# aoschu/esn-ofdm-mimo

Measured on AMD Instinct MI355X. Metric: OFDM symbols/s through the ESN detector (4x8 TDL-B, N=128, N_res=512; train+predict+detect), higher is better.
Workload: dtype f16 operands / f32 accumulate

## Files before the change

esn_ofdm_mimo_amd/build.py:

```python
import os
import subprocess
import sys

PKG = os.path.dirname(os.path.abspath(__file__))
CSRC = os.path.join(PKG, "csrc")
LIB = os.path.join(PKG, "libesn_hip.so")
SOURCES = ["esn_api.hip", "esn_host.hip", "esn_pack.hip", "esn_recur_f64.hip", "esn_recur_f64_mfma.hip", "esn_recur_mfma.hip",
           "esn_recur_big.hip", "esn_recur_cluster.hip", "esn_recur_mfma_f32.hip", "esn_recur_mfma_f16.hip", "esn_recur_mfma_bf16.hip", "esn_recur_skew16.hip", "esn_harvest_cluster.hip",
           "esn_solve_qr.hip", "esn_solve_chol.hip", "esn_solve_chol_big.hip", "esn_loo.hip", "esn_holdout.hip", "esn_gram.hip", "esn_detect.hip", "esn_remod.hip", "esn_gen.hip", "esn_reservoir.hip", "esn_specrad_split.hip", "esn_baseline.hip", "esn_chantrack.hip", "esn_chanstat.hip", "esn_coded.hip",
           "esn_elm.hip", "esn_fnn.hip"]
WITH_RS = os.environ.get("ESN_WITH_RS") == "1"
FLAGS = ["--offload-arch=gfx950", "-O3", "-std=c++17", "-fPIC", "-ffp-contract=off", "-fno-slp-vectorize",
         "-Wall", "-Wno-unused-function"]


def _stale():
    if not os.path.exists(LIB):
        return True
    t = os.path.getmtime(LIB)
    deps = [os.path.join(CSRC, f) for f in os.listdir(CSRC)] + \
           [os.path.join(PKG, "..", "include", "esn_hip.h"), os.path.abspath(__file__)]
    return any(os.path.getmtime(d) > t for d in deps)


def build_library(force=False, verbose=True, stamps=False):
    global LIB
    if stamps:
        extra = ["-DESN_STAMPS"] + os.environ.get("ESN_EXTRA_FLAGS", "").split()
        return _build(os.path.join(PKG, "libesn_hip_stamps.so"), "build_stamps", extra, verbose)
    if not force and not _stale():
        return LIB
    return _build(LIB, "build", [], verbose)


def _build(LIB, bdir, extra, verbose):
    hipcc = os.environ.get("HIPCC", "/opt/rocm/bin/hipcc")
    objs = []
    procs = []
    os.makedirs(os.path.join(PKG, bdir), exist_ok=True)
    sources = SOURCES + (["esn_recur_rs.hip"] if WITH_RS and LIB.endswith("_rs.so") else [])
    if len(sources) > len(SOURCES):
        extra = list(extra) + ["-DESN_WITH_RS"]
    for src in sources:
        obj = os.path.join(PKG, bdir, src.replace(".hip", ".o"))
        objs.append(obj)
        per_file = os.environ.get("ESN_FLAGS_" + src.replace(".hip", "").upper(), "").split()
        cmd = [hipcc, *FLAGS, *extra, *per_file, "-c", os.path.join(CSRC, src), "-o", obj]
        procs.append((src, subprocess.Popen(cmd, stdout=subprocess.PIPE, stderr=subprocess.STDOUT)))
    for src, pr in procs:
        out, _ = pr.communicate()
        if pr.returncode != 0:
            sys.stderr.write(out.decode())
            raise RuntimeError(f"hipcc failed on {src}")
        if verbose and out.strip():
            sys.stderr.write(out.decode())
    cmd = [hipcc, "--offload-arch=gfx950", "-shared", "-fPIC", "-o", LIB, *objs]
    subprocess.check_call(cmd)
    return LIB


if __name__ == "__main__":
    if "--variant" in sys.argv:
        name = sys.argv[sys.argv.index("--variant") + 1]
        print(_build(os.path.join(PKG, f"libesn_hip_{name}.so"), "build_" + name,
                     os.environ.get("ESN_EXTRA_FLAGS", "").split(), True))
    else:
        print(build_library(force="--force" in sys.argv, stamps="--stamps" in sys.argv))
```

esn_ofdm_mimo_amd/csrc/esn_api.hip:

```cpp
#include <stdarg.h>
#include <stdio.h>
#include <stdlib.h>
#include <math.h>
#include <string.h>
#include "esn_launch.h"
#include "esn_solve.h"

using namespace esn;

static thread_local char g_err[512] = "";

namespace esn {
int api_fail(int code, const char* fmt, ...) {
    va_list ap;
    va_start(ap, fmt);
    vsnprintf(g_err, sizeof(g_err), fmt, ap);
    va_end(ap);
    return code;
}
}
static int (&fail)(int, const char*, ...) = api_fail;

enum KnobRule {
    KNOB_FLAG,
    KNOB_INT,
    KNOB_TRIPLE,
    KNOB_BIG_NT,
    KNOB_HCLUSTER
};
struct KnobRow {
    const char* key;
    const char* env;
    size_t field;
    KnobRule rule;
    int dflt;
};
static const KnobRow kKnobTable[] = {
    {"skew", "ESN_SKEW", offsetof(Knobs, skew), KNOB_FLAG, 1},
    {"mfma_geom", "ESN_MFMA_GEOM", offsetof(Knobs, geom16), KNOB_TRIPLE, 0},
    {"mfma_geom_f32", "ESN_MFMA_GEOM_F32", offsetof(Knobs, geom32), KNOB_TRIPLE, 0},
    {"chol_skip", "ESN_CHOL_SKIP", offsetof(Knobs, chol_skip), KNOB_INT, 0},
    {"chol_dma", "ESN_CHOL_DMA", offsetof(Knobs, chol_dma), KNOB_FLAG, 1},
    {"f64_mfma", "ESN_F64_MFMA", offsetof(Knobs, f64_mfma), KNOB_FLAG, 1},
    {"rs", "ESN_RS", offsetof(Knobs, rs), KNOB_FLAG, 0},
    {"big_gemm", "ESN_BIG_GEMM", offsetof(Knobs, big_gemm), KNOB_FLAG, 1},
    {"cluster", "ESN_CLUSTER", offsetof(Knobs, cluster), KNOB_FLAG, 1},
    {"big_nt", "ESN_BIG_NT", offsetof(Knobs, big_nt), KNOB_BIG_NT, 2},
    {"big_pipe", "ESN_BIG_PIPE", offsetof(Knobs, big_pipe), KNOB_FLAG, 1},
    {"harvest_gemm", "ESN_HARVEST_GEMM", offsetof(Knobs, harvest_gemm), KNOB_FLAG, 0},
    {"gen_ko", nullptr, offsetof(Knobs, gen_ko), KNOB_INT, 0},
    {"s16", "ESN_S16", offsetof(Knobs, s16), KNOB_FLAG, 1},
    {"hcluster", "ESN_HCLUSTER", offsetof(Knobs, hcluster), KNOB_HCLUSTER, 1},
    {"detect_fixed", "ESN_DETECT_FIXED", offsetof(Knobs, detect_fixed), KNOB_FLAG, 1},
};

static void knob_parse(const KnobRow& r, const char* v, Knobs& k) {
    int* out = reinterpret_cast<int*>(reinterpret_cast<char*>(&k) + r.field);
    switch (r.rule) {
        case KNOB_FLAG: *out = (v && v[0] == '0' + !r.dflt) ? !r.dflt : r.dflt; break;
        case KNOB_INT: *out = v ? atoi(v) : r.dflt; break;
        case KNOB_TRIPLE: {
            int t[3];
            const bool ok = v && sscanf(v, "%d,%d,%d", &t[0], &t[1], &t[2]) == 3 && t[0] > 0 && t[1] > 0 && t[2] > 0;
            for (int i = 0; i < 3; ++i) out[i] = ok ? t[i] : 0;
            break;
        }
        case KNOB_BIG_NT: *out = (v && v[0] == '4') ? 4 : 2; break;
        case KNOB_HCLUSTER: *out = (v && (v[0] == '0' || v[0] == '4' || v[0] == '8')) ? v[0] - '0' : 1; break;
    }
}

namespace esn {
Knobs& knobs() {
    static Knobs k = [] {
        Knobs x{};
        for (const KnobRow& r : kKnobTable) knob_parse(r, r.env ? getenv(r.env) : nullptr, x);
        return x;
    }();
    return k;
}
}

static int hip_fail(int e, const char* what) {
    if (e == 0) return 0;
    if (e > 0) return fail(-1000 - e, "%s: HIP error %d (%s)", what, e, hipGetErrorString((hipError_t)e));
    return fail(-2, "%s: no kernel instance for this shape", what);
}

static bool check_shape(const esn_shape_t* s) {
    return s && s->n_res > 0 && s->n_in > 0 && s->n_out > 0 && s->n_wsets > 0;
}

static bool geometry_for(int precision, const esn_shape_t* s, Geometry* g, bool harvest = false) {
    memset(g, 0, sizeof(*g));
    if (precision == ESN_F64) {
        int fb = 8;
        while (fb > 1 && recur_f64_lds_bytes(fb, s->n_res, s->n_in, s->n_out) > 150 * 1024) fb >>= 1;
        if (recur_f64_lds_bytes(fb, s->n_res, s->n_in, s->n_out) > 160 * 1024) return false;
        Geometry gp, gh;
        memset(&gp, 0, sizeof(gp)); memset(&gh, 0, sizeof(gh));
        if (f64_mfma_geometry(s->n_res, s->n_in, s->n_out, false, &gp) &&
            f64_mfma_geometry(s->n_res, s->n_in, s->n_out, true, &gh))
            *g = harvest ? gh : gp;
        g->Bt = fb;
        return true;
    }
    if (precision < ESN_F64 || precision > ESN_BF16) return false;
    return mfma_geometry(precision, s->n_res, s->n_in, s->n_out, harvest, g);
}

#ifdef ESN_STAMPS
static unsigned long long* g_stamp_buf = nullptr;
extern "C" void esn_debug_set_stamp_buffer(void* dev) { g_stamp_buf = (unsigned long long*)dev; }
namespace esn { unsigned long long* stamp_buffer() { return g_stamp_buf; } }
#define ESN_SET_STAMPS(p) (p).stamps = g_stamp_buf
#else
#define ESN_SET_STAMPS(p) (p).stamps = nullptr
#endif

extern "C" {

const char* esn_last_error(void) { return g_err; }

int esn_abi_version(void) { return 10; }

int esn_debug_set(const char* key, const char* value) {
    if (!key) return fail(-1, "esn_debug_set: null key");
#ifndef ESN_WITH_RS
    if (!strcmp(key, "rs"))
        return (value && value[0] == '1')
                   ? fail(-3, "esn_debug_set: the register-state kernel is not in this build (ESN_WITH_RS=1)") : 0;
#endif
    for (const KnobRow& r : kKnobTable)
        if (!strcmp(key, r.key)) { knob_parse(r, value, knobs()); return 0; }
    return fail(-1, "esn_debug_set: unknown key '%s'", key);
}

int esn_device_info(int* cu_count, int* lds_bytes_per_cu, int* clock_khz, char* arch_name, int arch_name_len) {
    int dev = 0;
    hipError_t e = hipGetDevice(&dev);
    if (e != hipSuccess) return hip_fail((int)e, "hipGetDevice");
    hipDeviceProp_t prop;
    e = hipGetDeviceProperties(&prop, dev);
    if (e != hipSuccess) return hip_fail((int)e, "hipGetDeviceProperties");
    if (cu_count) *cu_count = prop.multiProcessorCount;
    if (lds_bytes_per_cu) *lds_bytes_per_cu = (int)prop.maxSharedMemoryPerMultiProcessor;
    if (clock_khz) *clock_khz = prop.clockRate;
    if (arch_name && arch_name_len > 0) {
        strncpy(arch_name, prop.gcnArchName, arch_name_len - 1);
        arch_name[arch_name_len - 1] = 0;
    }
    return 0;
}

int esn_tile_frames(int precision, const esn_shape_t* shape) {
    Geometry g;
    if (!check_shape(shape)) return fail(-1, "esn_tile_frames: invalid shape");
    if (!geometry_for(precision, shape, &g)) return fail(-2, "esn_tile_frames: unsupported shape/precision");
    return g.Bt;
}

size_t esn_packed_weights_bytes(int precision, const esn_shape_t* shape) {
    Geometry g;
    if (!check_shape(shape) || !geometry_for(precision, shape, &g)) return 0;
    return packed_w_bytes(precision, shape->n_res, shape->n_in, shape->n_out, g);
}

size_t esn_packed_readout_bytes(int precision, const esn_shape_t* shape) {
    Geometry g;
    if (!check_shape(shape) || !geometry_for(precision, shape, &g)) return 0;
    return packed_wout_bytes(precision, shape->n_res, shape->n_in, shape->n_out, g);
}

int esn_pack_weights(int precision, const esn_shape_t* shape, const double* W, const double* W_in,
                     const double* W_fb, void* packed, void* stream) {
    Geometry g;
    if (!check_shape(shape)) return fail(-1, "esn_pack_weights: invalid shape");
    if (!W || !W_in || !W_fb || !packed) return fail(-1, "esn_pack_weights: null pointer");
    if (!geometry_for(precision, shape, &g)) return fail(-2, "esn_pack_weights: unsupported shape/precision");
    return hip_fail(launch_pack_weights(precision, shape, g, W, W_in, W_fb, packed, (hipStream_t)stream),
                    "esn_pack_weights");
}

int esn_pack_readout(int precision, const esn_shape_t* shape, int n_groups, const double* W_out,
                     void* packed, void* stream) {
    Geometry g;
    if (!check_shape(shape) || n_groups <= 0) return fail(-1, "esn_pack_readout: invalid shape");
    if (!W_out || !packed) return fail(-1, "esn_pack_readout: null pointer");
    if (!geometry_for(precision, shape, &g)) return fail(-2, "esn_pack_readout: unsupported shape/precision");
    return hip_fail(launch_pack_readout(precision, shape, g, n_groups, W_out, packed, (hipStream_t)stream),
                    "esn_pack_readout");
}

static bool use_f64_mfma(int precision, const RecurParams& p) {
    return precision == ESN_F64 && p.g.m64 && p.n_frames > 8 && knobs().f64_mfma;
}

static int fill_common(RecurParams& p, int precision, const esn_shape_t* shape, const char* who,
                       bool harvest = false) {
    memset(&p, 0, sizeof(p));
    if (!check_shape(shape)) return fail(-1, "%s: invalid shape", who);
    if (!geometry_for(precision, shape, &p.g, harvest)) return fail(-2, "%s: unsupported shape/precision", who);
    p.n_res = shape->n_res; p.n_in = shape->n_in; p.n_out = shape->n_out;
    p.teacher_forcing = shape->teacher_forcing ? 1 : 0;
    p.n_wsets = shape->n_wsets;
    p.wset_stride = packed_w_bytes(precision, p.n_res, p.n_in, p.n_out, p.g);
    p.wout_stride = packed_wout_bytes(precision, p.n_res, p.n_in, p.n_out, p.g);
    p.leak = (shape->leak_rate == 0.0) ? 1.0 : shape->leak_rate;
    if (!(p.leak > 0.0 && p.leak <= 1.0)) return fail(-1, "%s: leak_rate %g outside (0, 1]", who, shape->leak_rate);
    if (p.leak != 1.0 && precision != ESN_F64)
        return fail(-2, "%s: leak_rate != 1 is an extension of the float64 kernels (precision ESN_F64)", who);
    p.w16_off = (size_t)p.g.Mp * p.g.Kp * 2;
    p.wo16_off = wout_big_offset(precision, p.n_out, p.g);
    p.w64_off = f64_w_offset(p.n_res, p.n_in, p.n_out);
    p.wo64_off = f64_wout_offset(p.n_res, p.n_in, p.n_out);
    p.harvest = harvest ? 1 : 0;
    return 0;
}

static void fill_batch(RecurParams& p, int precision, int n_frames, int frames_per_group) {
    p.n_frames = n_frames;
    p.F = frames_per_group;
    p.n_groups = (n_frames + frames_per_group - 1) / frames_per_group;
    const bool m64 = use_f64_mfma(precision, p);
    p.Fpad = p.harvest ? 1 : (precision == ESN_F64 && !m64) ? p.F : round_up(p.F, 16);
    if (precision == ESN_F64 && !m64 && (!p.harvest || p.n_wsets == 1)) {
        const long long slots = (long long)p.n_groups * p.Fpad;
        while (p.g.Bt > 1 && p.g.Bt / 2 >= slots) p.g.Bt >>= 1;
    }
    const int tile = m64 ? p.g.Bt64 : p.g.Bt;
    if (p.n_wsets > 1) {
        const int gpw = (p.n_groups + p.n_wsets - 1) / p.n_wsets;
        p.spw = round_up(gpw * p.Fpad, tile);
        p.n_tiles = p.n_wsets * (p.spw / tile);
    } else {
        p.n_tiles = (int)(((long long)p.n_groups * p.Fpad + tile - 1) / tile);
    }
}

struct Plan {
    int path;
    size_t workspace_bytes;
    int hc_members;
};
static bool path_uses_workspace(int path) {
    return path == ESN_PATH_CLUSTER_F64 || path == ESN_PATH_BIG_PREDICT || path == ESN_PATH_BIG_HARVEST ||
           path == ESN_PATH_HARVEST_CLUSTER;
}

static Plan plan_recur(int precision, const RecurParams& p, bool io32, bool workspace_lent) {
    const Knobs& k = knobs();
    const bool half = precision == ESN_F16 || precision == ESN_BF16;
    Plan pl = {ESN_PATH_MFMA, 0, 0};
    if (workspace_lent) {
        if (k.cluster && cluster_applies(precision, p))
            return {ESN_PATH_CLUSTER_F64, cluster_workspace_bytes(p.n_res, p.n_in, p.n_out, p.harvest != 0), 0};
        if (p.harvest && k.hcluster && harvest_cluster_applies(precision, p)) {
            const int members = k.hcluster == 1 ? 2 : k.hcluster;
            return {ESN_PATH_HARVEST_CLUSTER, harvest_cluster_workspace_bytes(p.n_groups, members, p.n_wsets), members};
        }
        if (p.harvest ? big_harvest_applies(precision, p) : (p.g.big && big_path_applies(precision, p))) {
            pl.workspace_bytes = p.harvest ? big_harvest_workspace_bytes(p.n_groups, p.g.Kp)
                                           : big_workspace_bytes(big_slots(p), p.g.Mp, p.g.Kp);
            if (k.big_gemm) { pl.path = p.harvest ? ESN_PATH_BIG_HARVEST : ESN_PATH_BIG_PREDICT; return pl; }
        }
    }
    if (!p.harvest) {
#ifdef ESN_WITH_RS
        if (!io32 && k.rs && rs_path_applies(precision, p) &&
            (size_t)p.n_frames * (p.S - p.transient) * p.n_out * 8 < 0x7fffffffu &&
            (size_t)p.n_groups * p.wout_stride < 0x7fffffffu) { pl.path = ESN_PATH_RS; return pl; }
#endif
        if (p.g.s16 && p.g.skew && k.s16 && half) { pl.path = ESN_PATH_SKEW16; return pl; }
    }
    (void)io32;
    pl.path = use_f64_mfma(precision, p) ? ESN_PATH_F64_MFMA : precision == ESN_F64 ? ESN_PATH_F64_VALU : ESN_PATH_MFMA;
    return pl;
}

static int launch_plan(const char* who, const char* size_query, int precision, RecurParams& p, bool io32,
                       void* workspace, size_t workspace_bytes, hipStream_t stream) {
    const Plan pl = plan_recur(precision, p, io32, workspace != nullptr);
    if (path_uses_workspace(pl.path) && workspace_bytes < pl.workspace_bytes)
        return fail(-1, "%s: workspace holds %zu bytes, %s says %zu", who, workspace_bytes, size_query,
                    pl.workspace_bytes);
    int e = -1;
    switch (pl.path) {
        case ESN_PATH_CLUSTER_F64: e = launch_recur_cluster(p, workspace, stream); break;
        case ESN_PATH_HARVEST_CLUSTER: e = launch_harvest_cluster(precision, p, pl.hc_members, workspace, stream); break;
        case ESN_PATH_BIG_HARVEST: e = launch_harvest_big(precision, p, workspace, stream); break;
        case ESN_PATH_BIG_PREDICT:
            p.Fpad = round_up(p.F, 16);
            e = launch_recur_big(precision, p, wout_big_offset(precision, p.n_out, p.g), workspace, stream, io32);
            break;
#ifdef ESN_WITH_RS
        case ESN_PATH_RS: e = launch_recur_rs(precision, p, wout_big_offset(precision, p.n_out, p.g), stream); break;
#endif
        case ESN_PATH_SKEW16: e = launch_recur_skew16(precision, p, stream, io32); break;
        case ESN_PATH_F64_MFMA: e = launch_recur_f64_mfma(p, stream); break;
        case ESN_PATH_F64_VALU: e = launch_recur_f64(p, stream); break;
        case ESN_PATH_MFMA: e = launch_recur_mfma(precision, p, stream, io32); break;
    }
    return hip_fail(e, who);
}

static int predict_common(const char* who, bool io32, int precision, const esn_shape_t* shape, const void* packed_w,
                          const void* packed_wout, const double* in_scale, const double* in_shift,
                          const double* t_scale, const double* t_shift, const void* U, int n_frames,
                          int frames_per_group, int T_in, int T, int transient, const double* x0, const double* y0,
                          double noise, int noise_mode, const double* noise_u, uint64_t seed, uint64_t group_offset,
                          void* Y, void* workspace, size_t workspace_bytes, void* stream) {
    if (io32 && precision == ESN_F64)
        return fail(-2, "%s: float32 I/O is served for precisions f32 / f16 / bf16; ESN_F64 reads and writes float64 "
                    "(esn_predict_batch)", who);
    RecurParams p;
    int rc = fill_common(p, precision, shape, who);
    if (rc) return rc;
    if (!packed_w || !packed_wout || !U || !Y) return fail(-1, "%s: null pointer", who);
    if (n_frames <= 0 || frames_per_group <= 0 || T <= 0 || T_in < 0 || T_in > T || transient < 0 || transient >= T)
        return fail(-1, "%s: invalid sizes (n_frames=%d F=%d T_in=%d T=%d transient=%d)",
                    who, n_frames, frames_per_group, T_in, T, transient);
    if (noise_mode == ESN_NOISE_TENSOR && !noise_u) return fail(-1, "%s: noise tensor missing", who);
    if (noise_mode < ESN_NOISE_NONE || noise_mode > ESN_NOISE_COUNTER) return fail(-1, "%s: bad noise mode", who);
    if (io32 && ((uintptr_t)U & ((shape->n_in & 3) == 0 ? 15 : 3)) != 0)
        return fail(-1, "%s: U must be %d-byte aligned", who, (shape->n_in & 3) == 0 ? 16 : 4);
    fill_batch(p, precision, n_frames, frames_per_group);
    p.T_in = T_in; p.S = T; p.in_row_off = 0; p.transient = transient;
    p.packed_w = packed_w; p.packed_wout = packed_wout;
    p.in_scale = in_scale; p.in_shift = in_shift; p.t_scale = t_scale; p.t_shift = t_shift;
    if (io32) p.U32 = static_cast<const float*>(U); else p.U = static_cast<const double*>(U);
    p.x0 = x0; p.y0 = y0; p.noise_u = noise_u;
    p.noise = noise; p.noise_mode = (noise == 0.0) ? ESN_NOISE_NONE : noise_mode; p.seed = seed;
    p.frame_off = (uint32_t)(group_offset * (uint64_t)frames_per_group);
    p.wset_rot = (int)(group_offset % (uint64_t)p.n_wsets);
    if (((uintptr_t)Y & 15) != 0) return fail(-1, "%s: Y must be 16-byte aligned", who);
    if (io32) p.Y32 = static_cast<float*>(Y); else p.Y = static_cast<double*>(Y);
    ESN_SET_STAMPS(p);
    return launch_plan(who, "esn_predict_workspace_bytes", precision, p, io32, workspace, workspace_bytes,
                       (hipStream_t)stream);
}

int esn_predict_batch(int precision, const esn_shape_t* shape, const void* packed_w, const void* packed_wout,
                      const double* in_scale, const double* in_shift, const double* t_scale,
                      const double* t_shift, const double* U, int n_frames, int frames_per_group, int T_in,
                      int T, int transient, const double* x0, const double* y0, double noise, int noise_mode,
                      const double* noise_u, uint64_t seed, uint64_t group_offset, double* Y, void* workspace,
                      size_t workspace_bytes, void* stream) {
    return predict_common("esn_predict_batch", false, precision, shape, packed_w, packed_wout, in_scale, in_shift,
                          t_scale, t_shift, U, n_frames, frames_per_group, T_in, T, transient, x0, y0, noise,
                          noise_mode, noise_u, seed, group_offset, Y, workspace, workspace_bytes, stream);
}

int esn_predict_batch_f32(int precision, const esn_shape_t* shape, const void* packed_w, const void* packed_wout,
                          const double* in_scale, const double* in_shift, const double* t_scale,
                          const double* t_shift, const float* U, int n_frames, int frames_per_group, int T_in,
                          int T, int transient, const double* x0, const double* y0, double noise, int noise_mode,
                          const double* noise_u, uint64_t seed, uint64_t group_offset, float* Y, void* workspace,
                          size_t workspace_bytes, void* stream) {
    return predict_common("esn_predict_batch_f32", true, precision, shape, packed_w, packed_wout, in_scale, in_shift,
                          t_scale, t_shift, U, n_frames, frames_per_group, T_in, T, transient, x0, y0, noise,
                          noise_mode, noise_u, seed, group_offset, Y, workspace, workspace_bytes, stream);
}

size_t esn_predict_workspace_bytes(int precision, const esn_shape_t* shape, int n_frames, int frames_per_group) {
    RecurParams p;
    if (n_frames <= 0 || frames_per_group <= 0) return 0;
    if (fill_common(p, precision, shape, "esn_predict_workspace_bytes")) return 0;
    fill_batch(p, precision, n_frames, frames_per_group);
    return plan_recur(precision, p, false, true).workspace_bytes;
}

size_t esn_harvest_workspace_bytes(int precision, const esn_shape_t* shape, int n_groups) {
    RecurParams p;
    if (n_groups <= 0) return 0;
    if (fill_common(p, precision, shape, "esn_harvest_workspace_bytes", true)) return 0;
    fill_batch(p, precision, n_groups, 1);
    return plan_recur(precision, p, false, true).workspace_bytes;
}

int esn_recur_path(int harvest, int precision, const esn_shape_t* shape, int n_sequences, int frames_per_group,
                   int have_workspace) {
    RecurParams p;
    int rc = fill_common(p, precision, shape, "esn_recur_path", harvest != 0);
    if (rc) return rc;
    if (harvest) frames_per_group = 1;
    if (n_sequences <= 0 || frames_per_group <= 0)
        return fail(-1, "esn_recur_path: invalid sizes (n_sequences=%d F=%d)", n_sequences, frames_per_group);
    fill_batch(p, precision, n_sequences, frames_per_group);
    return plan_recur(precision, p, false, have_workspace != 0).path;
}

static int harvest_common(int precision, const esn_shape_t* shape, const void* packed_w, const double* in_scale,
                      const double* in_shift, const double* t_scale, const double* t_shift, const double* U,
                      const double* D, int n_groups, int T, double noise, int noise_mode, const double* noise_u,
                      uint64_t seed, uint64_t group_offset, double* E, float* E32, void* workspace,
                      size_t workspace_bytes, void* stream) {
    RecurParams p;
    int rc = fill_common(p, precision, shape, "esn_harvest_batch", true);
    if (rc) return rc;
    if (!packed_w || !U || !D || (!E && !E32)) return fail(-1, "esn_harvest_batch: null pointer");
    if (E32 && precision == ESN_F64) return fail(-2, "esn_harvest_batch_f32: float32 states are an MFMA-kernel option (precision f32/f16/bf16)");
    if (n_groups <= 0 || T < 2) return fail(-1, "esn_harvest_batch: invalid sizes (n_groups=%d T=%d)", n_groups, T);
    if (noise_mode == ESN_NOISE_TENSOR && !noise_u) return fail(-1, "esn_harvest_batch: noise tensor missing");
    if (noise_mode < ESN_NOISE_NONE || noise_mode > ESN_NOISE_COUNTER) return fail(-1, "esn_harvest_batch: bad noise mode");
    fill_batch(p, precision, n_groups, 1);
    p.T_in = T; p.S = T - 1; p.in_row_off = 1; p.transient = 0;
    p.packed_w = packed_w;
    p.in_scale = in_scale; p.in_shift = in_shift; p.t_scale = t_scale; p.t_shift = t_shift;
    p.U = U; p.D = D; p.noise_u = noise_u;
    p.noise = noise; p.noise_mode = (noise == 0.0) ? ESN_NOISE_NONE : noise_mode; p.seed = seed;
    p.frame_off = (uint32_t)group_offset;
    p.wset_rot = (int)(group_offset % (uint64_t)p.n_wsets);
    if ((((uintptr_t)E) | ((uintptr_t)E32)) & 15) return fail(-1, "esn_harvest_batch: E must be 16-byte aligned");
    p.E = E; p.E32 = E32;
    ESN_SET_STAMPS(p);
    return launch_plan("esn_harvest_batch", "esn_harvest_workspace_bytes", precision, p, false, workspace,
                       workspace_bytes, (hipStream_t)stream);
}

int esn_harvest_batch(int precision, const esn_shape_t* shape, const void* packed_w, const double* in_scale,
                      const double* in_shift, const double* t_scale, const double* t_shift, const double* U,
                      const double* D, int n_groups, int T, double noise, int noise_mode, const double* noise_u,
                      uint64_t seed, uint64_t group_offset, double* E, void* workspace, size_t workspace_bytes,
                      void* stream) {
    if (!E) return fail(-1, "esn_harvest_batch: null pointer");
    return harvest_common(precision, shape, packed_w, in_scale, in_shift, t_scale, t_shift, U, D, n_groups, T, noise,
                          noise_mode, noise_u, seed, group_offset, E, nullptr, workspace, workspace_bytes, stream);
}

int esn_harvest_batch_f32(int precision, const esn_shape_t* shape, const void* packed_w, const double* in_scale,
                          const double* in_shift, const double* t_scale, const double* t_shift, const double* U,
                          const double* D, int n_groups, int T, double noise, int noise_mode,
                          const double* noise_u, uint64_t seed, uint64_t group_offset, float* E, void* workspace,
                          size_t workspace_bytes, void* stream) {
    if (!E) return fail(-1, "esn_harvest_batch_f32: null pointer");
    return harvest_common(precision, shape, packed_w, in_scale, in_shift, t_scale, t_shift, U, D, n_groups, T, noise,
                          noise_mode, noise_u, seed, group_offset, nullptr, E, workspace, workspace_bytes, stream);
}

size_t esn_readout_solve_workspace_bytes(int n_groups, int rows, int cols, int n_out) {
    if (n_groups <= 0 || rows <= 0 || cols <= 0 || n_out <= 0) return 0;
    return sizeof(double) * solve_work_doubles(rows, cols, n_out) * (size_t)n_groups;
// ... 742 lines not shown
```

esn_ofdm_mimo_amd/csrc/esn_harvest_cluster.hip:

```cpp
#include "esn_mfma_traits.h"
#include "esn_launch.h"

namespace esn {

constexpr int HC_NT = 256;
constexpr int HC_NKK = 17;
constexpr uint32_t HC_SPIN_LIMIT = 1u << 22;
constexpr unsigned long long HC_TAGMASK = 0x4000400040004000ULL;

static inline int hc_clusters(int n_pilots, int C, int n_wsets) {
    const int per_set = (n_pilots + n_wsets - 1) / n_wsets;
    return n_wsets * ((per_set + 8 * C - 1) / (8 * C));
}
size_t harvest_cluster_workspace_bytes(int n_pilots, int C, int n_wsets) {
    return (size_t)hc_clusters(n_pilots, C, n_wsets) * 2 * C * 8 * 1024 + 64;
}

__device__ __forceinline__ unsigned long long hc_tag_bits(int tag) {
    return ((unsigned long long)(tag & 1) << 14) | ((unsigned long long)((tag >> 1) & 1) << 30) |
           ((unsigned long long)((tag >> 2) & 1) << 46) | ((unsigned long long)((tag >> 3) & 1) << 62);
}

template <typename TR, int NOISE, int C>
__global__ __launch_bounds__(HC_NT) void harvest_cluster_kernel(RecurParams p, int n_clusters, unsigned long long* xch) {
    constexpr int ROWS = 512 / C;
    constexpr int RT = ROWS / 16, CT = C / 2;
    constexpr int P = 16 * CT;
    constexpr int NWC = CT < 2 ? CT : 2, NWR = 4 / NWC;
    constexpr int WR = RT / NWR, WC = CT / NWC;
    constexpr int KPM = ROWS / 32;
    constexpr int NG = (C - 1) * 2;
    constexpr int ZF_BYTES = CT * HC_NKK * 1024;
    constexpr int KREG = WR > 2 ? 12 : HC_NKK;
    constexpr int WL_WAVE = (HC_NKK - KREG) * WR * 1024;
    static_assert(RT % NWR == 0 && WR % 2 == 0 && CT * KPM == 8, "cluster shape");
    extern __shared__ __attribute__((aligned(16))) char hsm[];
    char* Zf = hsm;
    __shared__ int sh_dead;
    const int tid = threadIdx.x, lane = tid & 63;
    const int wave = __builtin_amdgcn_readfirstlane(tid >> 6);
    const int vr = wave / NWC, vc = wave % NWC;
    const int g4 = lane >> 4, col = lane & 15;
    const int lane16 = lane * 16;
    const Geometry& g = p.g;
    const int n_res = p.n_res, n_in = p.n_in, n_out = p.n_out;
    const int kin_p = g.kfb - g.kin;
    const int ncols = n_res + n_in;
    const int cpx = (n_clusters + 7) / 8;
    const int xcd = blockIdx.x & 7, li = blockIdx.x >> 3;
    const int cluster = xcd * cpx + li / C, c = li % C;
    if (cluster >= n_clusters) return;
    const int nws = p.n_wsets;
    const int ws = cluster % nws, kc = cluster / nws;
    const int gbase = (ws - p.wset_rot % nws + nws) % nws;
    unsigned int* err = reinterpret_cast<unsigned int*>(xch + (size_t)n_clusters * 2 * C * 1024);
    unsigned long long* xc = xch + (size_t)cluster * 2 * C * 1024;
    if (tid == 0) sh_dead = 0;

    u32x4 areg[KREG][WR];
    char* wl = hsm + ZF_BYTES + (size_t)wave * WL_WAVE + lane16;
    {
        const char* src = reinterpret_cast<const char*>(p.packed_w) + (size_t)ws * p.wset_stride + p.w16_off + lane16;
#pragma unroll
        for (int kk = 0; kk < HC_NKK; ++kk)
#pragma unroll
            for (int i = 0; i < WR; ++i) {
                const int grt = c * RT + vr * WR + i;
                const u32x4 f = *reinterpret_cast<const u32x4*>(src + ((size_t)((grt >> 2) * HC_NKK + kk) * 4 + (grt & 3)) * 1024);
                if (kk < KREG) areg[kk < KREG ? kk : 0][i] = f;
                else *reinterpret_cast<u32x4*>(wl + (size_t)((kk - KREG) * WR + i) * 1024) = f;
            }
        for (int i = tid; i < ZF_BYTES / 16; i += HC_NT) reinterpret_cast<u32x4*>(Zf)[i] = u32x4{0, 0, 0, 0};
    }
    auto pilot_of = [&](int f) -> int {
        const int gi = gbase + (kc * P + f) * nws;
        return gi < p.n_groups ? gi : -1;
    };
    auto store_E4 = [&](size_t idx, float v0, float v1, float v2, float v3) {
        if (p.E32) {
            *reinterpret_cast<f32x4*>(p.E32 + idx) = f32x4{v0, v1, v2, v3};
        } else {
            typedef double f64x2s __attribute__((ext_vector_type(2)));
            *reinterpret_cast<f64x2s*>(p.E + idx) = f64x2s{(double)v0, (double)v1};
            *reinterpret_cast<f64x2s*>(p.E + idx + 2) = f64x2s{(double)v2, (double)v3};
        }
    };
    constexpr int EPT = P / 8;
    const int sf = tid & (P - 1), sq = tid / P;
    const int s_pil = pilot_of(sf);
    const bool s_ok = s_pil >= 0;
    double uf_sc[EPT], uf_sh[EPT];
    int uf_kind[EPT];
#pragma unroll
    for (int e = 0; e < EPT; ++e) {
        const int pos = EPT * sq + e;
        uf_kind[e] = 0; uf_sc[e] = 0.0; uf_sh[e] = 0.0;
        if (!s_ok) continue;
        if (pos < n_in) {
            uf_kind[e] = 1;
            uf_sc[e] = p.in_scale ? p.in_scale[(size_t)s_pil * n_in + pos] : 1.0;
            uf_sh[e] = p.in_shift ? p.in_shift[(size_t)s_pil * n_in + pos] : 0.0;
        } else if (pos >= kin_p && pos < kin_p + n_out) {
            uf_kind[e] = 2;
            uf_sc[e] = p.t_scale ? p.t_scale[(size_t)s_pil * n_out + (pos - kin_p)] : 1.0;
            uf_sh[e] = p.t_shift ? p.t_shift[(size_t)s_pil * n_out + (pos - kin_p)] : 0.0;
        }
    }
    const double* uf_ptr[EPT];
    int uf_stride[EPT];
#pragma unroll
    for (int e = 0; e < EPT; ++e) {
        const int pos = EPT * sq + e;
        uf_ptr[e] = p.U; uf_stride[e] = 0;
        if (uf_kind[e] == 1) { uf_ptr[e] = p.U + ((size_t)s_pil * p.T_in + 1) * n_in + pos; uf_stride[e] = n_in; }
        if (uf_kind[e] == 2) { uf_ptr[e] = p.D + (size_t)s_pil * (p.S + 1) * n_out + (pos - kin_p); uf_stride[e] = n_out; }
    }
    auto fetch_uf = [&](int s, double (&raw)[EPT]) {
        const int sc = s < p.S ? s : p.S - 1;
#pragma unroll
        for (int e = 0; e < EPT; ++e) raw[e] = uf_ptr[e][(size_t)sc * uf_stride[e]];
    };
    auto stage_uf = [&](int s, const double (&raw)[EPT]) {
        uint32_t out[EPT / 2];
        double sv[EPT];
#pragma unroll
        for (int e = 0; e < EPT; ++e) sv[e] = uf_kind[e] ? raw[e] * uf_sc[e] + uf_sh[e] : 0.0;
#pragma unroll
        for (int e = 0; e < EPT / 2; ++e) out[e] = TR::pack2((float)sv[2 * e], (float)sv[2 * e + 1]);
        const int pos0 = EPT * sq;
        char* d = Zf + ((size_t)((sf >> 4) * HC_NKK + 16) * 64 + (pos0 >> 3) * 16 + (sf & 15)) * 16 + 2 * (pos0 & 7);
#pragma unroll
        for (int e = 0; e < EPT / 2; ++e) reinterpret_cast<uint32_t*>(d)[e] = out[e];
        if (c == 0 && s_ok && pos0 < n_in) {
            const size_t e0 = ((size_t)s_pil * (p.S + 1) + (s + 1)) * ncols + n_res + pos0;
#pragma unroll
            for (int e = 0; e < EPT; ++e)
                if (pos0 + e < n_in) { if (p.E32) p.E32[e0 + e] = (float)sv[e]; else p.E[e0 + e] = sv[e]; }
        }
    };
    if (c == 0 && s_ok && sq == 0) {
        const size_t e0 = (size_t)s_pil * (p.S + 1) * ncols;
        for (int k = 0; k < ncols; ++k) {
            double v = 0.0;
            if (k >= n_res) {
                const int ci = k - n_res;
                const double sc = p.in_scale ? p.in_scale[(size_t)s_pil * n_in + ci] : 1.0;
                const double sh = p.in_shift ? p.in_shift[(size_t)s_pil * n_in + ci] : 0.0;
                v = p.U[(size_t)s_pil * p.T_in * n_in + ci] * sc + sh;
            }
            if (p.E32) p.E32[e0 + k] = (float)v; else p.E[e0 + k] = v;
        }
    }
    __syncthreads();
    double raw_cur[EPT], raw_nx[EPT];
    fetch_uf(0, raw_cur);
    stage_uf(0, raw_cur);
    fetch_uf(1, raw_cur);

    const float noise = (float)p.noise;
    const float n_c1 = noise * (1.0f / 256.0f), n_c0 = noise * (0.5f / 256.0f - 0.5f);
    int fr2[WC];
    uint32_t key1[WC];
#pragma unroll
    for (int n = 0; n < WC; ++n) {
        const int pl = pilot_of((vc * WC + n) * 16 + col);
        fr2[n] = pl;
// ... 220 lines not shown
```

esn_ofdm_mimo_amd/csrc/esn_launch.h:

```cpp
#pragma once
#include "esn_common.h"

namespace esn {
int api_fail(int code, const char* fmt, ...);
#ifdef ESN_STAMPS
unsigned long long* stamp_buffer();
#endif
int launch_recur_f64(const RecurParams& p, hipStream_t stream);
size_t recur_f64_lds_bytes(int FB, int n_res, int n_in, int n_out);
bool f64_mfma_geometry(int n_res, int n_in, int n_out, bool harvest, Geometry* g);
int launch_recur_f64_mfma(const RecurParams& p, hipStream_t stream);
#ifdef ESN_WITH_RS
bool rs_path_applies(int precision, const RecurParams& p);
int launch_recur_rs(int precision, const RecurParams& p, size_t wo_rs_off, hipStream_t stream);
#endif
bool big_path_applies(int precision, const RecurParams& p);
int big_slots(const RecurParams& p);
size_t big_workspace_bytes(int n_slots, int Mp, int Kp);
size_t big_wout_image_bytes(int Mp);
int launch_recur_big(int precision, const RecurParams& p, size_t wo_big_off, void* workspace, hipStream_t stream,
                     bool io32 = false);
bool big_harvest_applies(int precision, const RecurParams& p);
size_t big_harvest_workspace_bytes(int n_groups, int Kp);
int launch_harvest_big(int precision, const RecurParams& p, void* workspace, hipStream_t stream);
bool cluster_applies(int precision, const RecurParams& p);
size_t cluster_workspace_bytes(int n_res, int n_in, int n_out, bool harvest);
int launch_recur_cluster(const RecurParams& p, void* workspace, hipStream_t stream);
bool mfma_geometry(int precision, int n_res, int n_in, int n_out, bool harvest, Geometry* g);
int launch_recur_mfma(int precision, const RecurParams& p, hipStream_t stream, bool io32 = false);
int launch_recur_mfma_f32(const RecurParams& p, hipStream_t stream, bool io32);
int launch_recur_mfma_f16(const RecurParams& p, hipStream_t stream, bool io32);
int launch_recur_mfma_bf16(const RecurParams& p, hipStream_t stream, bool io32);
bool harvest_cluster_applies(int precision, const RecurParams& p);
size_t harvest_cluster_workspace_bytes(int n_pilots, int C, int n_wsets);
int launch_harvest_cluster(int precision, const RecurParams& p, int C, void* workspace, hipStream_t stream);
int launch_recur_skew16(int precision, const RecurParams& p, hipStream_t stream, bool io32 = false);
size_t packed_w_bytes(int precision, int n_res, int n_in, int n_out, const Geometry& g);
size_t packed_wout_bytes(int precision, int n_res, int n_in, int n_out, const Geometry& g);
size_t wout_big_offset(int precision, int n_out, const Geometry& g);
size_t f64_w_offset(int n_res, int n_in, int n_out);
size_t f64_wout_offset(int n_res, int n_in, int n_out);
int launch_pack_weights(int precision, const esn_shape_t* sh, const Geometry& g, const double* W,
                        const double* Win, const double* Wfb, void* packed, hipStream_t stream);
int launch_pack_readout(int precision, const esn_shape_t* sh, const Geometry& g, int n_groups,
                        const double* Wout, void* packed, hipStream_t stream);
struct ReadoutArgs {
    const double* E; const float* E32; const double* D;
    int n_groups, T, transient, cols, n_out;
    const double *t_scale, *t_shift, *ridge; int n_ridge;
    double *W_out, *score; int *choice, *status;
    void* workspace; size_t workspace_bytes; hipStream_t stream;
};
int launch_readout_solve(const ReadoutArgs& a);
int launch_readout_chol(const ReadoutArgs& a);
int launch_readout_chol_big(const ReadoutArgs& a);
size_t ridge_loo_work_doubles();
int launch_ridge_loo(const ReadoutArgs& a);
struct HoldoutArgs {
    const double* E; const float* E32; const double* D; const double* W;
    int n_groups, T, transient, cols, n_out, n_ridge;
    const double *t_scale, *t_shift; const int* status_in;
    double* score; int* choice; hipStream_t stream;
};
int launch_holdout_score(const HoldoutArgs& a);
struct GramAccArgs {
    const double* E; const float* E32; const double* D;
    int n_groups, T, transient, cols, n_out;
    const double *t_scale, *t_shift; double decay;
    double *Gm, *Cm; hipStream_t stream;
};
struct GramSolveArgs {
    const double *Gm, *Cm; int n_groups, cols, n_out;
    const double* ridge; int n_ridge;
    double* W_out; int* status; void* workspace; size_t workspace_bytes; hipStream_t stream;
};
int gram_max_cols();
size_t gram_solve_work_doubles(int cols);
int launch_gram_accumulate(const GramAccArgs& a);
int launch_gram_solve(const GramSolveArgs& a);
size_t specrad_work_doubles(int n_res);
int launch_gen_reservoirs(int n_res, int n_in, int n_out, double sparsity, uint64_t seed, uint64_t first_set,
                          int n_sets, const double* uniforms, double* W, double* W_in, double* W_fb,
                          hipStream_t stream);
int launch_spectral_radius(const double* W, int n_sets, int n_res, int n_squarings, double* radius, int* status,
                           void* workspace, hipStream_t stream);
int launch_scale_reservoirs(double* W, int n_sets, int n_res, double rho, const double* radius, const int* status,
                            hipStream_t stream);
size_t specrad_split_work_bytes(int n_res);
int launch_spectral_radius_split(const double* W, int n_sets, int n_res, int n_squarings, double* radius, int* status,
                                 void* workspace, hipStream_t stream);
int launch_gen_taps(const TapParams& tp, hipStream_t stream);
int launch_gen_taps_doppler(const DopplerParams& dp, hipStream_t stream);
int launch_gen_frames(const FrameGenParams& fp, hipStream_t stream, bool c64 = false);
int launch_channel_estimate(const ChanEstParams& cp, hipStream_t stream);
int launch_mmse_detect(const MmseParams& mp, hipStream_t stream);
int launch_taps_to_freq(const TapsFreqParams& tp, hipStream_t stream);
int launch_channel_metrics(const ChanStatParams& cp, hipStream_t stream);
int launch_ldpc_encode(const LdpcEncodeParams& ep, hipStream_t stream);
int launch_qam_llr(const LlrParams& lp, hipStream_t stream);
int launch_ldpc_decode(const LdpcDecodeParams& dp, hipStream_t stream);
int launch_detect_count(const DetectParams& dp, hipStream_t stream, bool io32 = false);
int launch_detect_remod(const RemodParams& rp, hipStream_t stream);
int chantrack_segments(int n_sub, int n_t, int n_r);
size_t chantrack_lds_bytes(int n_sub, int n_t, int n_r, int isi);
int launch_channel_track(const ChanTrackParams& cp, hipStream_t stream);
int launch_elm_features(const ElmParams& p, hipStream_t stream);
int launch_elm_predict(int precision, const ElmParams& p, hipStream_t stream);
int launch_fnn_predict(int precision, const ElmParams& p, hipStream_t stream);
size_t fnn_train_lds_bytes(int n_in, int n_hidden, int window, int n_out, int T);
size_t fnn_train_workspace_bytes(int n_in, int n_hidden, int window, int n_groups);
int launch_fnn_train(const FnnTrainParams& p, hipStream_t stream);
}
```

Before: 12.35 million.

## Add single-block resident-weight harvest kernel as default harvest-cluster path

Adds a new harvest kernel in which one 256-thread block per 16 pilots holds the f16/bf16 reservoir weight fragments across accumulation registers, LDS slabs and a few L2 refetches for the whole time recursion. This replaces the multi-block cluster exchange that previously ran by default (members=2). With the default knob value 1 the new kernel is selected, so the cross-block synchronisation and workspace traffic of the cluster path go away. The cost is heavy register and LDS pressure and one block handling the full 512-wide state, which may limit parallelism or cause spills.

```diff
diff --git a/esn_ofdm_mimo_amd/build.py b/esn_ofdm_mimo_amd/build.py
--- a/esn_ofdm_mimo_amd/build.py
+++ b/esn_ofdm_mimo_amd/build.py
@@ -6,7 +6,7 @@
 CSRC = os.path.join(PKG, "csrc")
 LIB = os.path.join(PKG, "libesn_hip.so")
 SOURCES = ["esn_api.hip", "esn_host.hip", "esn_pack.hip", "esn_recur_f64.hip", "esn_recur_f64_mfma.hip", "esn_recur_mfma.hip",
-           "esn_recur_big.hip", "esn_recur_cluster.hip", "esn_recur_mfma_f32.hip", "esn_recur_mfma_f16.hip", "esn_recur_mfma_bf16.hip", "esn_recur_skew16.hip", "esn_harvest_cluster.hip",
+           "esn_recur_big.hip", "esn_recur_cluster.hip", "esn_recur_mfma_f32.hip", "esn_recur_mfma_f16.hip", "esn_recur_mfma_bf16.hip", "esn_recur_skew16.hip", "esn_harvest_cluster.hip", "esn_harvest_resident.hip",
            "esn_solve_qr.hip", "esn_solve_chol.hip", "esn_solve_chol_big.hip", "esn_loo.hip", "esn_holdout.hip", "esn_gram.hip", "esn_detect.hip", "esn_remod.hip", "esn_gen.hip", "esn_reservoir.hip", "esn_specrad_split.hip", "esn_baseline.hip", "esn_chantrack.hip", "esn_chanstat.hip", "esn_coded.hip",
            "esn_elm.hip", "esn_fnn.hip"]
 WITH_RS = os.environ.get("ESN_WITH_RS") == "1"
diff --git a/esn_ofdm_mimo_amd/csrc/esn_api.hip b/esn_ofdm_mimo_amd/csrc/esn_api.hip
--- a/esn_ofdm_mimo_amd/csrc/esn_api.hip
+++ b/esn_ofdm_mimo_amd/csrc/esn_api.hip
@@ -66,7 +66,7 @@
             break;
         }
         case KNOB_BIG_NT: *out = (v && v[0] == '4') ? 4 : 2; break;
-        case KNOB_HCLUSTER: *out = (v && (v[0] == '0' || v[0] == '4' || v[0] == '8')) ? v[0] - '0' : 1; break;
+        case KNOB_HCLUSTER: *out = (v && (v[0] == '0' || v[0] == '2' || v[0] == '4' || v[0] == '8')) ? v[0] - '0' : 1; break;
     }
 }
 
@@ -256,8 +256,9 @@
         if (k.cluster && cluster_applies(precision, p))
             return {ESN_PATH_CLUSTER_F64, cluster_workspace_bytes(p.n_res, p.n_in, p.n_out, p.harvest != 0), 0};
         if (p.harvest && k.hcluster && harvest_cluster_applies(precision, p)) {
-            const int members = k.hcluster == 1 ? 2 : k.hcluster;
-            return {ESN_PATH_HARVEST_CLUSTER, harvest_cluster_workspace_bytes(p.n_groups, members, p.n_wsets), members};
+            const int members = k.hcluster;
+            return {ESN_PATH_HARVEST_CLUSTER, harvest_cluster_workspace_bytes(p.n_groups, members == 1 ? 2 : members, p.n_wsets),
+                    members};
         }
         if (p.harvest ? big_harvest_applies(precision, p) : (p.g.big && big_path_applies(precision, p))) {
             pl.workspace_bytes = p.harvest ? big_harvest_workspace_bytes(p.n_groups, p.g.Kp)
@@ -287,7 +288,10 @@
     int e = -1;
     switch (pl.path) {
         case ESN_PATH_CLUSTER_F64: e = launch_recur_cluster(p, workspace, stream); break;
-        case ESN_PATH_HARVEST_CLUSTER: e = launch_harvest_cluster(precision, p, pl.hc_members, workspace, stream); break;
+        case ESN_PATH_HARVEST_CLUSTER:
+            e = pl.hc_members == 1 ? launch_harvest_resident(precision, p, workspace, stream)
+                                   : launch_harvest_cluster(precision, p, pl.hc_members, workspace, stream);
+            break;
         case ESN_PATH_BIG_HARVEST: e = launch_harvest_big(precision, p, workspace, stream); break;
         case ESN_PATH_BIG_PREDICT:
             p.Fpad = round_up(p.F, 16);
diff --git a/esn_ofdm_mimo_amd/csrc/esn_harvest_cluster.hip b/esn_ofdm_mimo_amd/csrc/esn_harvest_cluster.hip
--- a/esn_ofdm_mimo_amd/csrc/esn_harvest_cluster.hip
+++ b/esn_ofdm_mimo_amd/csrc/esn_harvest_cluster.hip
@@ -12,6 +12,7 @@
     const int per_set = (n_pilots + n_wsets - 1) / n_wsets;
     return n_wsets * ((per_set + 8 * C - 1) / (8 * C));
 }
+int harvest_cluster_count(int n_pilots, int C, int n_wsets) { return hc_clusters(n_pilots, C, n_wsets); }
 size_t harvest_cluster_workspace_bytes(int n_pilots, int C, int n_wsets) {
     return (size_t)hc_clusters(n_pilots, C, n_wsets) * 2 * C * 8 * 1024 + 64;
 }
diff --git a/esn_ofdm_mimo_amd/csrc/esn_harvest_resident.hip b/esn_ofdm_mimo_amd/csrc/esn_harvest_resident.hip
--- /dev/null
+++ b/esn_ofdm_mimo_amd/csrc/esn_harvest_resident.hip
@@ -0,0 +1,306 @@
+#include "esn_mfma_traits.h"
+#include "esn_launch.h"
+
+namespace esn {
+
+constexpr int HR_NT = 256;
+constexpr int HR_NKK = 17;
+constexpr int HR_WR = 8;
+constexpr int HR_P = 16;
+constexpr int HR_ZF_BYTES = HR_NKK * 1024;
+constexpr int HR_NLDS = 35;
+constexpr int HR_NXTRA = HR_NLDS - 2 * HR_NKK;
+constexpr int HR_WL_WAVE = HR_NLDS * 1024;
+static_assert(HR_NXTRA >= 0 && HR_NXTRA <= HR_NKK, "slab shape");
+constexpr unsigned int HR_LDS_BYTES = HR_ZF_BYTES + 4 * HR_WL_WAVE;
+static_assert(HR_LDS_BYTES <= 160 * 1024, "LDS of one CU");
+extern "C" __device__ __attribute__((used)) const unsigned int esn_harvest_resident_lds = HR_LDS_BYTES;
+constexpr int HR_BQ = 3;
+constexpr int HR_ML2 = 2;
+constexpr int HR_LEAD = 4;
+__host__ __device__ constexpr int hr_nl2(int noise) { return noise == ESN_NOISE_TENSOR ? 12 : 4; }
+constexpr int HR_KACC = 9;
+
+__host__ __device__ constexpr int hr_slot(int kk, int m) {
+    return (m & 3) == 3 ? 2 * kk + (m >> 2)
+         : (m == 6 && kk >= HR_NKK - HR_NXTRA) ? 2 * HR_NKK + (kk - (HR_NKK - HR_NXTRA)) : -1;
+}
+__host__ __device__ constexpr bool hr_from_l2(int nl2, int kk, int m) { return m == HR_ML2 && kk >= HR_NKK - nl2; }
+__host__ __device__ constexpr int hr_l2_issue(int kk) { return kk > HR_LEAD ? kk - HR_LEAD : 0; }
+
+template <typename TR, int NOISE>
+__global__ __launch_bounds__(HR_NT) void harvest_resident_kernel(RecurParams p, int n_clusters) {
+    constexpr int NL2 = hr_nl2(NOISE);
+    extern __shared__ __attribute__((aligned(16))) char hsm[];
+    char* Zf = hsm;
+    const int tid = threadIdx.x, lane = tid & 63;
+    const int wave = __builtin_amdgcn_readfirstlane(tid >> 6);
+    const int g4 = lane >> 4, col = lane & 15;
+    const int lane16 = lane * 16;
+    const Geometry& g = p.g;
+    const int n_res = p.n_res, n_in = p.n_in, n_out = p.n_out;
+    const int kin_p = g.kfb - g.kin;
+    const int ncols = n_res + n_in;
+    const int cluster = blockIdx.x;
+    if (cluster >= n_clusters) return;
+    const int nws = p.n_wsets;
+    const int ws = cluster % nws, kc = cluster / nws;
+    const int gbase = (ws - p.wset_rot % nws + nws) % nws;
+
+    auto pilot_of = [&](int f) -> int {
+        const int gi = gbase + (kc * HR_P + f) * nws;
+        return gi < p.n_groups ? gi : -1;
+    };
+    auto store_E4 = [&](size_t idx, float v0, float v1, float v2, float v3) {
+        if (p.E32) {
+            *reinterpret_cast<f32x4*>(p.E32 + idx) = f32x4{v0, v1, v2, v3};
+        } else {
+            typedef double f64x2s __attribute__((ext_vector_type(2)));
+            *reinterpret_cast<f64x2s*>(p.E + idx) = f64x2s{(double)v0, (double)v1};
+            *reinterpret_cast<f64x2s*>(p.E + idx + 2) = f64x2s{(double)v2, (double)v3};
+        }
+    };
+    constexpr int EPT = 2;
+    const int sf = tid & (HR_P - 1), sq = tid / HR_P;
+    const int s_pil = pilot_of(sf);
+    const bool s_ok = s_pil >= 0;
+    const int pos0 = EPT * sq;
+    double uf_sc[EPT], uf_sh[EPT];
+    const double* uf_ptr = p.U;
+    int uf_stride = 0, uf_two = 0;
+#pragma unroll
+    for (int e = 0; e < EPT; ++e) { uf_sc[e] = 0.0; uf_sh[e] = 0.0; }
+    if (s_ok && pos0 < n_in) {
+        uf_ptr = p.U + ((size_t)s_pil * p.T_in + 1) * n_in + pos0; uf_stride = n_in; uf_two = 1;
+#pragma unroll
+        for (int e = 0; e < EPT; ++e) {
+            uf_sc[e] = p.in_scale ? p.in_scale[(size_t)s_pil * n_in + pos0 + e] : 1.0;
+            uf_sh[e] = p.in_shift ? p.in_shift[(size_t)s_pil * n_in + pos0 + e] : 0.0;
+        }
+    } else if (s_ok && pos0 >= kin_p && pos0 < kin_p + n_out) {
+        uf_ptr = p.D + (size_t)s_pil * (p.S + 1) * n_out + (pos0 - kin_p); uf_stride = n_out;
+        uf_two = pos0 + 1 < kin_p + n_out ? 1 : 0;
+#pragma unroll
+        for (int e = 0; e <= uf_two; ++e) {
+            uf_sc[e] = p.t_scale ? p.t_scale[(size_t)s_pil * n_out + (pos0 + e - kin_p)] : 1.0;
+            uf_sh[e] = p.t_shift ? p.t_shift[(size_t)s_pil * n_out + (pos0 + e - kin_p)] : 0.0;
+        }
+    }
+    auto fetch_uf = [&](int s, double (&raw)[EPT]) {
+        const int sc = s < p.S ? s : p.S - 1;
+        const double* src = uf_ptr + (size_t)sc * uf_stride;
+        raw[0] = src[0];
+        raw[1] = src[uf_two];
+    };
+    auto stage_uf = [&](int s, const double (&raw)[EPT]) {
+        double sv[EPT];
+        sv[0] = uf_stride ? raw[0] * uf_sc[0] + uf_sh[0] : 0.0;
+        sv[1] = uf_two ? raw[1] * uf_sc[1] + uf_sh[1] : 0.0;
+        char* d = Zf + ((size_t)16 * 64 + (pos0 >> 3) * 16 + sf) * 16 + 2 * (pos0 & 7);
+        *reinterpret_cast<uint32_t*>(d) = TR::pack2((float)sv[0], (float)sv[1]);
+        if (s_ok && pos0 < n_in) {
+            const size_t e0 = ((size_t)s_pil * (p.S + 1) + (s + 1)) * ncols + n_res + pos0;
+#pragma unroll
+            for (int e = 0; e < EPT; ++e) { if (p.E32) p.E32[e0 + e] = (float)sv[e]; else p.E[e0 + e] = sv[e]; }
+        }
+    };
+    u32x4 areg[HR_NKK][HR_WR];
+    char* wl = hsm + HR_ZF_BYTES + (size_t)wave * HR_WL_WAVE + lane16;
+    const char* wsrc = reinterpret_cast<const char*>(p.packed_w) + (size_t)ws * p.wset_stride + p.w16_off;
+    auto frag = [&](int kk, int m) -> u32x4 {
+        const int grt = wave * HR_WR + m;
+        return *reinterpret_cast<const u32x4*>(wsrc + ((size_t)((grt >> 2) * HR_NKK + kk) * 4 + (grt & 3)) * 1024 + lane16);
+    };
+    {
+#pragma unroll
+        for (int kk = 0; kk < HR_NKK; ++kk)
+#pragma unroll
+            for (int m = 0; m < HR_WR; ++m) {
+                if (hr_from_l2(NL2, kk, m)) continue;
+                const u32x4 f = frag(kk, m);
+                if (hr_slot(kk, m) < 0) areg[kk][m] = f;
+                else *reinterpret_cast<u32x4*>(wl + (size_t)hr_slot(kk, m) * 1024) = f;
+            }
+#pragma unroll
+        for (int kk = 0; kk < HR_NKK; ++kk)
+#pragma unroll
+            for (int m = 0; m < HR_WR; ++m)
+                if (kk < HR_KACC && hr_slot(kk, m) < 0 && !hr_from_l2(NL2, kk, m)) asm volatile("" : "+a"(areg[kk][m]));
+        for (int i = tid; i < HR_ZF_BYTES / 16; i += HR_NT) reinterpret_cast<u32x4*>(Zf)[i] = u32x4{0, 0, 0, 0};
+    }
+    for (int i = tid; i < HR_P * ncols; i += HR_NT) {
+        const int pl = pilot_of(i / ncols), k = i % ncols;
+        if (pl < 0) continue;
+        double v = 0.0;
+        if (k >= n_res) {
+            const int ci = k - n_res;
+            const double sc = p.in_scale ? p.in_scale[(size_t)pl * n_in + ci] : 1.0;
+            const double sh = p.in_shift ? p.in_shift[(size_t)pl * n_in + ci] : 0.0;
+            v = p.U[(size_t)pl * p.T_in * n_in + ci] * sc + sh;
+        }
+        const size_t e0 = (size_t)pl * (p.S + 1) * ncols;
+        if (p.E32) p.E32[e0 + k] = (float)v; else p.E[e0 + k] = v;
+    }
+    __syncthreads();
+    double raw[EPT];
+    fetch_uf(0, raw);
+    stage_uf(0, raw);
+
+    const float noise = (float)p.noise;
+    const float n_c1 = noise * (1.0f / 256.0f), n_c0 = noise * (0.5f / 256.0f - 0.5f);
+    const int fr2 = pilot_of(col);
+    const uint32_t key1 = mix32((uint32_t)p.seed ^ (((uint32_t)fr2 + p.frame_off) * 0x9E3779B9U));
+    const uint32_t seed_hi = (uint32_t)(p.seed >> 32);
+    __syncthreads();
+
+    const char* zf_w = Zf + lane16;
+#ifdef ESN_STAMPS
+    unsigned long long hst[4] = {0, 0, 0, 0};
+#define HR_T(v) const unsigned long long v = __builtin_amdgcn_s_memrealtime();
+#else
+#define HR_T(v)
+#endif
+    auto gemm_half = [&](auto m0c, f32x4 (&acc)[4], auto between) {
+        constexpr int M0 = decltype(m0c)::value;
+        u32x4 bq[HR_BQ], l2f[HR_NKK], wq[2][4];
+#pragma unroll
+        for (int i = 0; i < 4; ++i) acc[i] = f32x4{0.f, 0.f, 0.f, 0.f};
+#pragma unroll
+        for (int i = 0; i < 4; ++i)
+            if (hr_slot(0, M0 + i) >= 0) wq[0][i] = *reinterpret_cast<const u32x4*>(wl + (size_t)hr_slot(0, M0 + i) * 1024);
+#pragma unroll
+        for (int j = 0; j < HR_BQ; ++j) bq[j] = *reinterpret_cast<const u32x4*>(zf_w + (size_t)j * 1024);
+#pragma unroll
+        for (int kk = 0; kk < HR_NKK; ++kk) {
+            u32x4 af[4];
+            if (HR_ML2 >= M0 && HR_ML2 < M0 + 4) {
+#pragma unroll
+                for (int ku = kk; ku < HR_NKK; ++ku)
+                    if (hr_from_l2(NL2, ku, HR_ML2) && hr_l2_issue(ku) == kk) l2f[ku] = frag(ku, HR_ML2);
+            }
+            if (kk + 1 < HR_NKK) {
+#pragma unroll
+                for (int i = 0; i < 4; ++i)
+                    if (hr_slot(kk + 1, M0 + i) >= 0)
+                        wq[(kk + 1) & 1][i] = *reinterpret_cast<const u32x4*>(wl + (size_t)hr_slot(kk + 1, M0 + i) * 1024);
+            }
+#pragma unroll
+            for (int i = 0; i < 4; ++i) {
+                if (hr_from_l2(NL2, kk, M0 + i)) af[i] = l2f[kk];
+                else if (hr_slot(kk, M0 + i) < 0) af[i] = areg[kk][M0 + i];
+                else af[i] = wq[kk & 1][i];
+                TR::mma16(acc[i], af[i], bq[kk % HR_BQ]);
+            }
+            if (kk + HR_BQ < HR_NKK) bq[kk % HR_BQ] = *reinterpret_cast<const u32x4*>(zf_w + (size_t)(kk + HR_BQ) * 1024);
+            between(kk);
+            __builtin_amdgcn_sched_barrier(0);
+        }
+    };
+    for (int s = 0; s < p.S; ++s) {
+        HR_T(ht0)
+        fetch_uf(s + 1, raw);
+        const uint32_t step_mix = seed_hi ^ ((uint32_t)s * 0x85EBCA6BU + 0x27d4eb2fU);
+        uint32_t key = 0;
+        const double* nz = nullptr;
+        if (NOISE == ESN_NOISE_COUNTER) key = mix32(key1 ^ step_mix) + (uint32_t)((16 * HR_WR * wave) / 4 + g4) * 0x9E3779B9U;
+        if (NOISE == ESN_NOISE_TENSOR && fr2 >= 0) nz = p.noise_u + ((size_t)fr2 * p.S + s) * n_res;
+        auto finish_tile = [&](int m, float (&v)[4], uint32_t& w0, uint32_t& w1) {
+            const int row = 16 * (HR_WR * wave + m) + 4 * g4;
+            if (NOISE == ESN_NOISE_COUNTER) {
+                const uint32_t sq4 = noise_mix(key + (uint32_t)(4 * m) * 0x9E3779B9U);
+                v[0] = fmaf((float)(sq4 & 0xffU), n_c1, v[0] + n_c0);
+                v[1] = fmaf((float)((sq4 >> 8) & 0xffU), n_c1, v[1] + n_c0);
+                v[2] = fmaf((float)((sq4 >> 16) & 0xffU), n_c1, v[2] + n_c0);
+                v[3] = fmaf((float)(sq4 >> 24), n_c1, v[3] + n_c0);
+            } else if (NOISE == ESN_NOISE_TENSOR) {
+#pragma unroll
+                for (int j = 0; j < 4; ++j)
+                    if (nz && row + j < n_res) v[j] += noise * ((float)nz[row + j] - 0.5f);
+            }
+            w0 = TR::pack2(v[0], v[1]);
+            w1 = TR::pack2(v[2], v[3]);
+            if (fr2 >= 0 && row < n_res) {
+                float r[4];
+                TR::unpack2(w0, r[0], r[1]);
+                TR::unpack2(w1, r[2], r[3]);
+                store_E4(((size_t)fr2 * (p.S + 1) + (s + 1)) * ncols + row, r[0], r[1], r[2], r[3]);
+            }
+        };
+        f32x4 acc0[4], acc1[4];
+        uint32_t out0[2][4];
+        float v0[4];
+        gemm_half(std::integral_constant<int, 0>{}, acc0, [&](int) {});
+        gemm_half(std::integral_constant<int, 4>{}, acc1, [&](int kk) {
+            if (kk < 16) {
+                v0[kk & 3] = TR::act(acc0[kk >> 2][kk & 3]);
+                if ((kk & 3) == 3) finish_tile(kk >> 2, v0, out0[kk >> 3][2 * ((kk >> 2) & 1)], out0[kk >> 3][2 * ((kk >> 2) & 1) + 1]);
+            }
+        });
+        HR_T(ht1)
+        __syncthreads();
+        HR_T(ht2)
+#pragma unroll
+        for (int pr = 0; pr < 2; ++pr)
+            *reinterpret_cast<u32x4*>(Zf + ((size_t)((HR_WR / 2) * wave + pr) * 64 + lane) * 16) =
+                u32x4{out0[pr][0], out0[pr][1], out0[pr][2], out0[pr][3]};
+#pragma unroll
+        for (int pr = 2; pr < HR_WR / 2; ++pr) {
+            uint32_t outw[4];
+#pragma unroll
+            for (int tt = 0; tt < 2; ++tt) {
+                const int m = 2 * pr + tt;
+                float v[4];
+#pragma unroll
+                for (int j = 0; j < 4; ++j) v[j] = TR::act(acc1[m - 4][j]);
+                finish_tile(m, v, outw[2 * tt], outw[2 * tt + 1]);
+            }
+            *reinterpret_cast<u32x4*>(Zf + ((size_t)((HR_WR / 2) * wave + pr) * 64 + lane) * 16) =
+                u32x4{outw[0], outw[1], outw[2], outw[3]};
+            __builtin_amdgcn_sched_barrier(0);
+        }
+        HR_T(ht3)
+        if (s + 1 == p.S) break;
+        stage_uf(s + 1, raw);
+        __syncthreads();
+#ifdef ESN_STAMPS
+        {
+            const unsigned long long ht4 = __builtin_amdgcn_s_memrealtime();
+            hst[0] += ht1 - ht0; hst[1] += ht2 - ht1; hst[2] += ht3 - ht2; hst[3] += ht4 - ht3;
+        }
+#endif
+    }
+#ifdef ESN_STAMPS
+    if (p.stamps && blockIdx.x == 0 && lane == 0) {
+        for (int i = 0; i < 4; ++i) p.stamps[wave * 8 + i] = hst[i];
+        p.stamps[wave * 8 + 7] = 1;
+    }
+#endif
+}
+
+template <typename TR>
+static int launch_hr(const RecurParams& p, int n_clusters, hipStream_t stream) {
+    const size_t lds = HR_LDS_BYTES;
+    auto go = [&](auto kern) -> int {
+        hipError_t e = hipFuncSetAttribute(reinterpret_cast<const void*>(kern), hipFuncAttributeMaxDynamicSharedMemorySize, (int)lds);
+        if (e != hipSuccess) return (int)e;
+        hipLaunchKernelGGL(kern, dim3(n_clusters), dim3(HR_NT), lds, stream, p, n_clusters);
+        return (int)hipGetLastError();
+    };
+    switch (p.noise_mode) {
+        case ESN_NOISE_NONE: return go(harvest_resident_kernel<TR, ESN_NOISE_NONE>);
+        case ESN_NOISE_TENSOR: return go(harvest_resident_kernel<TR, ESN_NOISE_TENSOR>);
+        default: return go(harvest_resident_kernel<TR, ESN_NOISE_COUNTER>);
+    }
+}
+
+int launch_harvest_resident(int precision, const RecurParams& p, void* workspace, hipStream_t stream) {
+    const int n_clusters = harvest_cluster_count(p.n_groups, 2, p.n_wsets);
+    char* err = reinterpret_cast<char*>(workspace) + harvest_cluster_workspace_bytes(p.n_groups, 2, p.n_wsets) - 64;
+    hipError_t e = hipMemsetAsync(err, 0, 64, stream);
+    if (e != hipSuccess) return (int)e;
+    if (precision == ESN_F16) return launch_hr<TraitsF16>(p, n_clusters, stream);
+    if (precision == ESN_BF16) return launch_hr<TraitsBF16>(p, n_clusters, stream);
+    return -1;
+}
+
+}
diff --git a/esn_ofdm_mimo_amd/csrc/esn_launch.h b/esn_ofdm_mimo_amd/csrc/esn_launch.h
--- a/esn_ofdm_mimo_amd/csrc/esn_launch.h
+++ b/esn_ofdm_mimo_amd/csrc/esn_launch.h
@@ -32,8 +32,10 @@
 int launch_recur_mfma_f16(const RecurParams& p, hipStream_t stream, bool io32);
 int launch_recur_mfma_bf16(const RecurParams& p, hipStream_t stream, bool io32);
 bool harvest_cluster_applies(int precision, const RecurParams& p);
+int harvest_cluster_count(int n_pilots, int C, int n_wsets);
 size_t harvest_cluster_workspace_bytes(int n_pilots, int C, int n_wsets);
 int launch_harvest_cluster(int precision, const RecurParams& p, int C, void* workspace, hipStream_t stream);
+int launch_harvest_resident(int precision, const RecurParams& p, void* workspace, hipStream_t stream);
 int launch_recur_skew16(int precision, const RecurParams& p, hipStream_t stream, bool io32 = false);
 size_t packed_w_bytes(int precision, int n_res, int n_in, int n_out, const Geometry& g);
 size_t packed_wout_bytes(int precision, int n_res, int n_in, int n_out, const Geometry& g);
```

New measurement: 12.47 million (median of 6 runs). About the same (+1.0%).
